# debbiemarkslab/BEAR

Measured on AMD Instinct MI355X. Metric: k-mer contexts/sec (DM-marginal+grad h), k=13, higher is better.
Workload: dtype f64

## Files before the change

### bear_amd/csrc/bear_hip.hip

```cpp
#include "bear_host.h"
#include "kernels_finalize.h"
#include "kernels_rows.h"
#include "kernels_sorted.h"
#include "kernels_plan.h"
#include "kernels_synth.h"
#include "kernels_refmix.h"
#include "kernels_mixplan.h"
#include "kernels_sample.h"
#include "kernels_shuffle.h"
#include "kernels_refplan.h"

#ifdef PLN_STAMPS
#define PLN_DBG_ARG , ws->dbg
#else
#define PLN_DBG_ARG
#endif

thread_local int g_last_hip_error = 0;

extern "C" {

int bear_abi_version(void) { return BEAR_ABI_VERSION; }

const char *bear_strerror(int status) {
// ... 451 lines not shown
  (void)hipSetDevice(prev);
  if (e != hipSuccess) {
    g_last_hip_error = (int)e;
    return BEAR_ERR_HIP;
  }
  for (uint64_t k = 0; k < count; ++k) {
    row0[k] = h[k].row0;
    rows[k] = h[k].rows_items >> 16;
    items[k] = h[k].rows_items & 0xffffu;
    stream_offset[k] = (uint64_t)h[k].off16 * 16;
  }
  return BEAR_OK;
}

int bear_plan_create_ref(bear_ws *ws, const uint32_t *train, const uint32_t *ref, uint64_t n_rows, bear_plan **out) {
  if (!out) return BEAR_ERR_INVALID_ARG;
  *out = nullptr;
  if ((n_rows && !ref) || misaligned(ref)) return BEAR_ERR_INVALID_ARG;
  bear_plan *p = nullptr;
  int st = bear_plan_create(ws, train, n_rows, 4, &p);
  if (st != BEAR_OK) return st;
  p->ref = ref;
  if (p->count_total[1] > 0.0 && (double)p->n_heavy[0] * 2.0 > p->count_total[1]) {
    (void)hipFree(p->tiles);
    (void)hipFree(p->stream);
    (void)hipFree(p->heavy_col);
    (void)hipFree(p->heavy_row);
    (void)hipFree(p->heavy_stop);
    p->tiles = nullptr;
    p->stream = nullptr;
    p->heavy_col = nullptr;
    p->heavy_row = nullptr;
    p->heavy_stop = nullptr;
    p->n_tiles = 0;
    p->n_heavy[0] = p->n_heavy[1] = p->n_heavy[2] = 0;
    p->rows_ref = 1;
    p->bytes = sizeof(unsigned long long) * (2 * SRT_NKEY + PLN_NBIG + 1);
    *out = p;
    return BEAR_OK;
  }
  unsigned long long *d_meta = nullptr;
  hipError_t e = hipMalloc(&d_meta, sizeof(unsigned long long) * 72);
  if (e == hipSuccess) e = hipMemset(d_meta, 0, sizeof(unsigned long long) * 72);
  if (e == hipSuccess) e = hipMalloc(&p->sum0, sizeof(double));
  if (e == hipSuccess) e = hipMemset(p->sum0, 0, sizeof(double));
  p->hist0_base = d_meta;
  unsigned long long h_meta[72];
  memset(h_meta, 0, sizeof(h_meta));
  const int grid = grid_capped((n_rows + 1023) / 1024, (uint64_t)ws->num_cu * 8);
  if (e == hipSuccess && n_rows) {
    hipLaunchKernelGGL(rpl_build_kernel, dim3(grid), dim3(256), 0, 0, train, ref, n_rows, 0, d_meta, d_meta + 32, d_meta + 64, p->sum0,
                       static_cast<rpl_item *>(nullptr), static_cast<uint32_t *>(nullptr));
    e = hipGetLastError();
    if (e == hipSuccess) e = hipMemcpy(h_meta, d_meta, sizeof(h_meta), hipMemcpyDeviceToHost);
  }
  if (e == hipSuccess) {
    unsigned long long run = 0, cur[RPL_NKEY];
    for (int k = 0; k < RPL_NKEY; ++k) {
      cur[k] = run;
      run += h_meta[k];
    }
    p->n_ref_items = run;
    p->n_heavy0 = h_meta[64];
    if (run) e = hipMalloc(&p->ref_items, sizeof(rpl_item) * run);
    if (e == hipSuccess && p->n_heavy0) e = hipMalloc(&p->heavy0, sizeof(uint32_t) * p->n_heavy0);
    if (e == hipSuccess) e = hipMemcpy(d_meta, cur, sizeof(cur), hipMemcpyHostToDevice);
    if (e == hipSuccess) e = hipMemset(d_meta + 64, 0, sizeof(unsigned long long));
    if (e == hipSuccess && n_rows && (run || p->n_heavy0)) {
      hipLaunchKernelGGL(rpl_build_kernel, dim3(grid), dim3(256), 0, 0, train, ref, n_rows, 1, d_meta, d_meta + 32, d_meta + 64, p->sum0,
                         p->ref_items, p->heavy0);
      e = hipGetLastError();
    }
    if (e == hipSuccess) e = hipDeviceSynchronize();
#ifdef BEAR_DET_BUILD
    for (int k = 0; k < RPL_NKEY && e == hipSuccess; ++k)
      if (bear_canonical_order(p->ref_items + cur[k], h_meta[k], 16, 0) != BEAR_OK) e = hipErrorUnknown;
    if (e == hipSuccess && bear_canonical_order(p->heavy0, p->n_heavy0, 4, 0) != BEAR_OK) e = hipErrorUnknown;
#endif
  }
  if (e != hipSuccess) {
    g_last_hip_error = (int)e;
    plan_free(p);
    return e == hipErrorOutOfMemory ? BEAR_ERR_NOMEM : BEAR_ERR_HIP;
  }
  p->hist0 = d_meta + 32;
  p->bytes += sizeof(rpl_item) * p->n_ref_items + sizeof(uint32_t) * p->n_heavy0 + sizeof(unsigned long long) * 72;
  *out = p;
  return BEAR_OK;
}

static int launch_prior_plan(bear_ws *ws, const bear_plan *plan, const double *prior, uint64_t n_rows, const bear_params &prm,
                             const double *theta, int train_ar, int prior_normalized, double *out, hipStream_t s) {
  const int grid = grid_plan(ws, plan->n_tiles);
  const double2 *lt = reinterpret_cast<const double2 *>(ws->logtab);
  const bear_step_io io = ws_io(ws, theta, BEAR_THETA_NET, out);
  if (train_ar)
    hipLaunchKernelGGL((dm_prior_plan_kernel<true, true>), dim3(grid), dim3(PLN_THREADS), sizeof(pln_lds_n), s, prior, n_rows, prm,
                       plan_view(plan), lt, ws->partials, io PLN_DBG_ARG);
  else if (prior_normalized)
    hipLaunchKernelGGL((dm_prior_plan_kernel<true, false>), dim3(grid), dim3(PLN_THREADS), sizeof(pln_lds_n), s, prior, n_rows, prm,
                       plan_view(plan), lt, ws->partials, io PLN_DBG_ARG);
  else
    hipLaunchKernelGGL((dm_prior_plan_kernel<false, false>), dim3(grid), dim3(PLN_THREADS), sizeof(pln_lds_n), s, prior, n_rows, prm,
                       plan_view(plan), lt, ws->partials, io PLN_DBG_ARG);
  HIP_TRY(hipGetLastError());
  return BEAR_OK;
}

int bear_dm_prior_plan_f64(bear_ws *ws, const bear_plan *plan, const uint32_t *counts, const double *prior,
                           uint64_t n_rows, double h_signed, double eps, int train_ar, int prior_normalized,
                           double *out, void *stream) {
  int st = check_ws(ws);
  if (st != BEAR_OK) return st;
  if (!plan || !out || (n_rows && (!counts || !prior))) return BEAR_ERR_INVALID_ARG;
  if (check_plan_step(ws, plan, counts, n_rows, 5, true) != BEAR_OK || misaligned(prior) || misaligned8(out)) return BEAR_ERR_INVALID_ARG;
  const bear_params prm = params_net(h_signed, eps);
  if (plan_is_rows(plan)) return launch_prior_rows(ws, plan, prior, prm, nullptr, train_ar, out, nullptr, static_cast<hipStream_t>(stream));
  return launch_prior_plan(ws, plan, prior, n_rows, prm, nullptr, train_ar, prior_normalized, out, static_cast<hipStream_t>(stream));
}

int launch_prior_plan_grad(bear_ws *ws, const bear_plan *plan, const double *prior, const bear_params &prm,
                                  const double *theta, int train_ar, int prior_normalized, double *out, double *grad_prior,
                                  hipStream_t s) {
  const int grid = grid_plan(ws, plan->n_tiles);
  const double2 *lt = reinterpret_cast<const double2 *>(ws->logtab);
  const pln_view pv = plan_view(plan);
  const bear_step_io io = ws_io(ws, theta, BEAR_THETA_NET, out);
  if (train_ar)
    hipLaunchKernelGGL((dm_prior_plan_grad_kernel<true, true>), dim3(grid), dim3(PLN_THREADS), sizeof(pln_lds_g), s, prior, prm, pv, lt,
                       grad_prior, ws->partials, io);
  else if (prior_normalized)
    hipLaunchKernelGGL(dm_prior_plan_grad_inplace_kernel, dim3(grid), dim3(PLN_THREADS), sizeof(pln_lds_gi), s, prior, prm, pv, lt,
                       grad_prior, ws->partials, io);
  else
    hipLaunchKernelGGL((dm_prior_plan_grad_kernel<false, false>), dim3(grid), dim3(PLN_THREADS), sizeof(pln_lds_g), s, prior, prm, pv, lt,
                       grad_prior, ws->partials, io);
  HIP_TRY(hipGetLastError());
  auto fixup_grid = [&](uint64_t nh) { return grid_capped((nh + 255) / 256, (uint64_t)ws->num_cu * 8); };
#define FIXUP(NORM, AR, ROWS, N) \
  hipLaunchKernelGGL((dm_prior_grad_fixup_kernel<NORM, AR, ROWS>), dim3(fixup_grid(N)), dim3(256), 0, s, prior, prm, pv, lt, grad_prior, io)
  if (pv.n_heavy_row && !train_ar) {
    if (prior_normalized) FIXUP(true, false, true, pv.n_heavy_row);
    else FIXUP(false, false, true, pv.n_heavy_row);
  }
  if (pv.n_heavy_col) {
    if (train_ar) FIXUP(true, true, false, pv.n_heavy_col);
    else if (prior_normalized) FIXUP(true, false, false, pv.n_heavy_col);
    else FIXUP(false, false, false, pv.n_heavy_col);
  }
#undef FIXUP
  HIP_TRY(hipGetLastError());
  return BEAR_OK;
}

int bear_dm_prior_plan_grad_f64(bear_ws *ws, const bear_plan *plan, const uint32_t *counts, const double *prior,
                                uint64_t n_rows, double h_signed, double eps, int train_ar, int prior_normalized,
                                double *out, double *grad_prior, void *stream) {
  int st = check_ws(ws);
  if (st != BEAR_OK) return st;
  if (!plan || !out || !grad_prior || (n_rows && (!counts || !prior))) return BEAR_ERR_INVALID_ARG;
  if (check_plan_step(ws, plan, counts, n_rows, 5, true) != BEAR_OK) return BEAR_ERR_INVALID_ARG;
  if (misaligned(prior) || misaligned(grad_prior) || misaligned8(out)) return BEAR_ERR_INVALID_ARG;
  const bear_params prm = params_net(h_signed, eps);
  if (plan_is_rows(plan)) return launch_prior_rows(ws, plan, prior, prm, nullptr, train_ar, out, grad_prior, static_cast<hipStream_t>(stream));
  return launch_prior_plan_grad(ws, plan, prior, prm, nullptr, train_ar, prior_normalized, out, grad_prior,
                                static_cast<hipStream_t>(stream));
}

int bear_dm_prior_plan_dev_f64(bear_ws *ws, const bear_plan *plan, const uint32_t *counts, const double *prior, uint64_t n_rows,
                               const double *h_signed_dev, double eps, int train_ar, int prior_normalized, double *out,
                               double *grad_prior, void *stream) {
  int st = check_ws(ws);
  if (st != BEAR_OK) return st;
  if (!plan || !out || !h_signed_dev || (n_rows && (!counts || !prior))) return BEAR_ERR_INVALID_ARG;
  if (check_plan_step(ws, plan, counts, n_rows, 5, true) != BEAR_OK) return BEAR_ERR_INVALID_ARG;
  if (misaligned(prior) || misaligned(grad_prior) || misaligned8(out)) return BEAR_ERR_INVALID_ARG;
  hipStream_t s = static_cast<hipStream_t>(stream);
  const bear_params only_eps = params_eps(eps);
  if (plan_is_rows(plan)) return launch_prior_rows(ws, plan, prior, only_eps, h_signed_dev, train_ar, out, grad_prior, s);
  if (grad_prior) return launch_prior_plan_grad(ws, plan, prior, only_eps, h_signed_dev, train_ar, prior_normalized, out, grad_prior, s);
  return launch_prior_plan(ws, plan, prior, n_rows, only_eps, h_signed_dev, train_ar, prior_normalized, out, s);
}

int bear_dm_refmix_plan_grad_f64(bear_ws *ws, const bear_plan *plan, const uint32_t *counts, const double *net_rows,
                                 const double *ref_rows, uint64_t n_rows, const double *h_signed_dev, const double *tau_signed_dev,
                                 const double *net_weight_signed_dev, double eps, int train_ar, double *out, double *grad_net_rows,
                                 void *stream) {
  int st = check_ws(ws);
  if (st != BEAR_OK) return st;
  if (!plan || !out || !h_signed_dev || !tau_signed_dev || !net_weight_signed_dev) return BEAR_ERR_INVALID_ARG;
  if (n_rows && (!counts || !net_rows || !ref_rows || !grad_net_rows)) return BEAR_ERR_INVALID_ARG;
  if (check_plan_step(ws, plan, counts, n_rows, 5) != BEAR_OK) return BEAR_ERR_INVALID_ARG;
  if (misaligned(net_rows) || misaligned(ref_rows) || misaligned(grad_net_rows) || misaligned8(out) || misaligned8(h_signed_dev) ||
      misaligned8(tau_signed_dev) || misaligned8(net_weight_signed_dev) || !(eps >= 0.0))
    return BEAR_ERR_INVALID_ARG;
  hipStream_t s = static_cast<hipStream_t>(stream);
  const int grid = grid_plan(ws, plan->n_tiles);
  const double2 *lt = reinterpret_cast<const double2 *>(ws->logtab);
  const pln_view pv = plan_view(plan);
  const bear_step_io io = ws_io(ws, nullptr, BEAR_THETA_REF, out);
#define MIX_LAUNCH(AR)                                                                                                            \
  hipLaunchKernelGGL(dm_refmix_plan_grad_kernel<AR>, dim3(grid), dim3(PLN_THREADS), sizeof(pln_lds_g), s, net_rows, ref_rows, \
                     h_signed_dev, tau_signed_dev, net_weight_signed_dev, eps, pv, lt, grad_net_rows, ws->partials, io)
  BEAR_DISPATCH_1(train_ar, MIX_LAUNCH);
#undef MIX_LAUNCH
  HIP_TRY(hipGetLastError());
  if (pv.n_heavy_col + pv.n_heavy_row) {
    const uint64_t nh = pv.n_heavy_col + pv.n_heavy_row;
    const int g2 = grid_capped((nh + 255) / 256, (uint64_t)ws->num_cu * 4);
#define MIX_FIXUP(AR)                                                                                                      \
  hipLaunchKernelGGL(dm_refmix_fixup_kernel<AR>, dim3(g2), dim3(256), 0, s, net_rows, ref_rows, h_signed_dev, tau_signed_dev, \
                     net_weight_signed_dev, eps, pv, lt, grad_net_rows)
    BEAR_DISPATCH_1(train_ar, MIX_FIXUP);
#undef MIX_FIXUP
    HIP_TRY(hipGetLastError());
  }
  return BEAR_OK;
}


static int launch_ref_plan(bear_ws *ws, const bear_plan *plan, const uint32_t *ref, uint64_t n_rows, const bear_params &prm,
                           const double *theta, int train_ar, double *out, hipStream_t s, const bear_apply_io &apply = NO_APPLY) {
  const double2 *lt = reinterpret_cast<const double2 *>(ws->logtab);
  const bear_step_io io = ws_io(ws, theta, BEAR_THETA_REF, out);
  int grid;
  if (plan->rows_ref) {
    if (plan->ref != ref) return BEAR_ERR_INVALID_ARG;
    grid = grid_dense(ws, n_rows);
#define REF_ROWS(AR) \
  hipLaunchKernelGGL(dm_ref_rows_kernel<AR>, dim3(grid), dim3(BEAR_THREADS), 0, s, plan->counts, ref, n_rows, prm, lt, ws->partials, io, apply)
    BEAR_DISPATCH_1(train_ar, REF_ROWS);
#undef REF_ROWS
  } else if (plan->ref) {
    if (plan->ref != ref) return BEAR_ERR_INVALID_ARG;
    rpl_view rv;
    rv.items = plan->ref_items;
    rv.n_items = plan->n_ref_items;
    rv.hist0 = plan->hist0;
    rv.heavy0 = plan->heavy0;
    rv.n_heavy0 = plan->n_heavy0;
    rv.sum0 = plan->sum0;
    const uint64_t units = (plan->n_ref_items + 63) / 64, want = (units + 3) / 4 + 2, cap = (uint64_t)ws->num_cu * (units > 131072 ? 6 : 4);
    grid = grid_capped(want, cap);
#define REF_ITEMS(AR) \
  hipLaunchKernelGGL(dm_ref_items_kernel<AR>, dim3(grid), dim3(256), 0, s, prm, rv, plan_view(plan), lt, ws->partials, io, apply)
    BEAR_DISPATCH_1(train_ar, REF_ITEMS);
#undef REF_ITEMS
  } else {
    grid = grid_plan(ws, plan->n_tiles);
#define REF_PLAN(AR)                                                                                                                     \
  hipLaunchKernelGGL(dm_ref_plan_kernel<AR>, dim3(grid), dim3(PLN_THREADS), sizeof(pln_lds_r), s, ref, n_rows, prm, plan_view(plan), lt, \
                     ws->partials, io, apply)
    BEAR_DISPATCH_1(train_ar, REF_PLAN);
#undef REF_PLAN
  }
  HIP_TRY(hipGetLastError());
  return BEAR_OK;
}

int bear_dm_ref_plan_f64(bear_ws *ws, const bear_plan *plan, const uint32_t *train, const uint32_t *ref,
                         uint64_t n_rows, double h_signed, double tau_signed, double nu_signed, double eps,
                         int train_ar, double *out, void *stream) {
  int st = check_ws(ws);
  if (st != BEAR_OK) return st;
  if (!plan || !out || (n_rows && (!train || !ref))) return BEAR_ERR_INVALID_ARG;
  if (check_plan_step(ws, plan, train, n_rows, 4) != BEAR_OK || misaligned(ref) || misaligned8(out)) return BEAR_ERR_INVALID_ARG;
  return launch_ref_plan(ws, plan, ref, n_rows, params_ref(h_signed, tau_signed, nu_signed, eps), nullptr, train_ar, out,
                         static_cast<hipStream_t>(stream));
}

static int ref_reduce(bear_ws *ws, const bear_plan *plan, const uint32_t *train, const uint32_t *ref, uint64_t n_rows, const double *theta,
                      double eps, int train_ar, double *packed, hipStream_t s, const bear_apply_io &apply) {
  int st = check_ws(ws);
  if (st != BEAR_OK) return st;
  if (!plan || !packed || !theta || !n_rows || !train || !ref) return BEAR_ERR_INVALID_ARG;
  if (check_plan_step(ws, plan, train, n_rows, 4) != BEAR_OK || misaligned(ref) || misaligned8(packed)) return BEAR_ERR_INVALID_ARG;
  return launch_ref_plan(ws, plan, ref, n_rows, params_eps(eps), theta, train_ar, packed, s, apply);
}

int bear_ref_train_reduce_f64(bear_ws *ws, const bear_plan *plan, const uint32_t *train, const uint32_t *ref, uint64_t n_rows,
                              const double *theta, double eps, int train_ar, double *packed, void *stream) {
  return ref_reduce(ws, plan, train, ref, n_rows, theta, eps, train_ar, packed, static_cast<hipStream_t>(stream), NO_APPLY);
}

int bear_ref_train_step_f64(bear_ws *ws, const bear_plan *plan, const uint32_t *train, const uint32_t *ref, uint64_t n_rows,
                            double *theta, double *adam_m, double *adam_v, double *adam_t, double eps, int train_ar,
                            double learning_rate, double scale, double *out, double *loss_buf, uint64_t loss_cap, void *stream) {
  if (!adam_m || !adam_v || !adam_t) return BEAR_ERR_INVALID_ARG;
  hipStream_t s = static_cast<hipStream_t>(stream);
  if (two_launch_step()) {
    int st = ref_reduce(ws, plan, train, ref, n_rows, theta, eps, train_ar, out, s, NO_APPLY);
    if (st != BEAR_OK) return st;
    return launch_train_apply(theta, 3, out, adam_m, adam_v, adam_t, learning_rate, scale, train_ar, loss_buf, loss_cap, s);
  }
  return ref_reduce(ws, plan, train, ref, n_rows, theta, eps, train_ar, out, s,
                    make_apply(theta, 3, adam_m, adam_v, adam_t, learning_rate, scale, train_ar, loss_buf, loss_cap));
}

int bear_dm_items_f64(bear_ws *ws, const double *x, const uint32_t *c, uint64_t n, int path, double *D, double *P,
                      void *stream) {
  int st = check_ws(ws);
  if (st != BEAR_OK) return st;
  if (n == 0) return BEAR_OK;
  if (!x || !c || !D || !P || path < 0 || path > 2) return BEAR_ERR_INVALID_ARG;
  uint64_t blocks = (n + 255) / 256;
  if (blocks > 0x7fffffffull) return BEAR_ERR_INVALID_ARG;
  hipLaunchKernelGGL(dm_items_kernel, dim3((unsigned)blocks), dim3(256), 0, static_cast<hipStream_t>(stream), x, c, n, path,
                     reinterpret_cast<const double2 *>(ws->logtab), D, P);
  HIP_TRY(hipGetLastError());
  return BEAR_OK;
}

int bear_plan_count_total(const bear_plan *plan, double *total, double *bound) {
  if (!plan) return BEAR_ERR_INVALID_ARG;
  for (int k = 0; k < 3; ++k) {
    if (total) total[k] = plan->count_total[k];
    if (bound) bound[k] = plan->count_bound[k];
  }
  return BEAR_OK;
}

int bear_plan_set_count_bound(bear_plan *plan, const double *bound) {
  if (!plan || !bound) return BEAR_ERR_INVALID_ARG;
  for (int k = 0; k < 3; ++k)
    if (!(bound[k] >= plan->count_total[k]) || !(bound[k] < 0x1p50)) return BEAR_ERR_INVALID_ARG;
  for (int k = 0; k < 3; ++k) plan->count_bound[k] = bound[k];
  return BEAR_OK;
}

static int refmix_grid(const bear_ws *ws, uint64_t n_rows) { return grid_capped((n_rows + RMX_THREADS - 1) / RMX_THREADS, ws_blocks(ws, 2)); }

int bear_ref_mix_forward_f64(bear_ws *ws, const double *net_rows, const double *ref_rows, uint64_t n_rows, const double *tau_signed,
                             const double *net_weight_signed, double *prior, void *stream) {
  int st = check_ws(ws);
  if (st != BEAR_OK) return st;
  if (!tau_signed || !net_weight_signed || misaligned8(tau_signed) || misaligned8(net_weight_signed)) return BEAR_ERR_INVALID_ARG;
  if (n_rows == 0) return BEAR_OK;
  if (!net_rows || !ref_rows || !prior || misaligned(net_rows) || misaligned(ref_rows) || misaligned(prior)) return BEAR_ERR_INVALID_ARG;
  hipLaunchKernelGGL(ref_mix_forward_kernel, dim3(refmix_grid(ws, n_rows)), dim3(RMX_THREADS), 0, static_cast<hipStream_t>(stream),
                     net_rows, ref_rows, tau_signed, net_weight_signed, n_rows, prior);
  HIP_TRY(hipGetLastError());
  return BEAR_OK;
}

int bear_ref_mix_backward_f64(bear_ws *ws, const double *net_rows, const double *ref_rows, const double *grad_prior, uint64_t n_rows,
                              const double *tau_signed, const double *net_weight_signed, double *grad_net_rows, double *grad_scalars,
                              void *stream) {
  int st = check_ws(ws);
  if (st != BEAR_OK) return st;
  if (!tau_signed || !net_weight_signed || !grad_scalars || misaligned8(tau_signed) || misaligned8(net_weight_signed) ||
      misaligned8(grad_scalars))
    return BEAR_ERR_INVALID_ARG;
  hipStream_t s = static_cast<hipStream_t>(stream);
  if (n_rows == 0) {
    HIP_TRY(hipMemsetAsync(grad_scalars, 0, 2 * sizeof(double), s));
    return BEAR_OK;
  }
  if (!net_rows || !ref_rows || !grad_prior || !grad_net_rows || misaligned(net_rows) || misaligned(ref_rows) ||
      misaligned(grad_prior) || misaligned(grad_net_rows))
    return BEAR_ERR_INVALID_ARG;
  hipLaunchKernelGGL(ref_mix_backward_kernel, dim3(refmix_grid(ws, n_rows)), dim3(RMX_THREADS), 0, s, net_rows, ref_rows, grad_prior,
                     tau_signed, net_weight_signed, n_rows, grad_net_rows, ws->partials, ws_arrival(ws), grad_scalars);
  HIP_TRY(hipGetLastError());
  return BEAR_OK;
}

int bear_debug_read_timing(bear_ws *ws, unsigned long long *host, int n_words) {
  if (!ws || !host) return BEAR_ERR_INVALID_ARG;
  HIP_TRY(hipDeviceSynchronize());
  HIP_TRY(hipMemcpy(host, ws->dbg, sizeof(unsigned long long) * (size_t)n_words, hipMemcpyDeviceToHost));
  return BEAR_OK;
}

int bear_debug_occupancy(int which) {
  int nb = -1;
  hipError_t e = which == 0
      ? hipOccupancyMaxActiveBlocksPerMultiprocessor(&nb, dm_prior_sorted_kernel<0>, SRT_THREADS, sizeof(srt_lds_n))
      : hipOccupancyMaxActiveBlocksPerMultiprocessor(&nb, dm_ref_sorted_kernel, SRT_THREADS, sizeof(srt_lds_r));
  return e == hipSuccess ? nb : -1000 - (int)e;
}

int bear_log_gamma_f64(const double *conc, uint64_t n, uint64_t n_samples, uint64_t seed, double *out, void *stream) {
  if (n == 0 || n_samples == 0) return BEAR_OK;
  if (!conc || !out) return BEAR_ERR_INVALID_ARG;
  if (n_samples > (~0ull) / n) return BEAR_ERR_INVALID_ARG;
  const uint64_t total = n * n_samples;
  uint64_t blocks = (total + SMP_THREADS - 1) / SMP_THREADS;
  if (blocks > 65536) blocks = 65536;
  hipLaunchKernelGGL(log_gamma_kernel, dim3((unsigned)blocks), dim3(SMP_THREADS), 0, static_cast<hipStream_t>(stream), conc, n,
                     n_samples, seed, out);
  HIP_TRY(hipGetLastError());
  return BEAR_OK;
}

static int logdir_sample_launch(const uint32_t *counts, const double *prior, uint64_t n_rows, int width, const double *h,
                                int n_h, int with_ar, const double *van, int n_van, int mc_samples, int map, uint64_t seed,
                                uint64_t row_base, double *out, void *stream) {
  if (n_h < 0 || n_van < 0 || n_h + n_van > SMP_MAX_MODELS || (n_h && !h) || (n_van && !van)) return BEAR_ERR_INVALID_ARG;
  if (with_ar && !map) return BEAR_ERR_INVALID_ARG;
  if (map) mc_samples = 1;
  if (mc_samples <= 0) return BEAR_ERR_INVALID_ARG;
  const int M = (with_ar ? 1 : 0) + n_h + n_van;
  if (n_rows == 0 || M == 0) return BEAR_OK;
  if (!out || ((n_h || with_ar) && !prior)) return BEAR_ERR_INVALID_ARG;
  smp_args A;
  memset(&A, 0, sizeof(A));
  A.n_h = n_h;
  A.n_van = n_van;
  A.arm = with_ar ? 1 : 0;
  A.has_counts = counts ? 1 : 0;
  A.has_prior = prior ? 1 : 0;
  A.map = map ? 1 : 0;
  A.mc = (uint32_t)mc_samples;
  A.seed = seed;
  A.row_base = row_base;
  for (int j = 0; j < n_h; ++j) {
    if (!(h[j] > 0.0)) return BEAR_ERR_INVALID_ARG;
    A.w[j] = 1.0 / h[j];
  }
  for (int k = 0; k < n_van; ++k) A.w[n_h + k] = van[k];
  const uint64_t per_row = (uint64_t)M * (uint64_t)mc_samples;
  if (per_row > 0xffffffffull || n_rows > (~0ull) / ((uint64_t)width * per_row)) return BEAR_ERR_INVALID_ARG;
  uint64_t blocks = (n_rows * per_row + SMP_THREADS - 1) / SMP_THREADS;
  if (blocks > 65536) blocks = 65536;
  hipStream_t s = static_cast<hipStream_t>(stream);
  if (width == 21)
    hipLaunchKernelGGL(logdir_sample_kernel<21>, dim3((unsigned)blocks), dim3(SMP_THREADS), 0, s, counts, prior, n_rows, A, out);
  else
    hipLaunchKernelGGL(logdir_sample_kernel<5>, dim3((unsigned)blocks), dim3(SMP_THREADS), 0, s, counts, prior, n_rows, A, out);
  HIP_TRY(hipGetLastError());
  return BEAR_OK;
}

int bear_logdir_sample_f64(const uint32_t *counts, const double *prior, uint64_t n_rows, const double *h, int n_h,
                           int with_ar, const double *van, int n_van, int mc_samples, int map, uint64_t seed,
                           uint64_t row_base, double *out, void *stream) {
  return logdir_sample_launch(counts, prior, n_rows, 5, h, n_h, with_ar, van, n_van, mc_samples, map, seed, row_base, out, stream);
}

int bear_logdir_sample_wide_f64(const uint32_t *counts, const double *prior, uint64_t n_rows, int width, const double *h,
                                int n_h, int with_ar, const double *van, int n_van, int mc_samples, int map, uint64_t seed,
                                uint64_t row_base, double *out, void *stream) {
  if (!wide_width_ok(width)) return BEAR_ERR_INVALID_ARG;
  return logdir_sample_launch(counts, prior, n_rows, width, h, n_h, with_ar, van, n_van, mc_samples, map, seed, row_base, out,
                              stream);
}

int bear_shuffle_rows(const void *src, void *dst, uint64_t n_rows, uint32_t row_bytes, uint64_t seed, void *stream) {
  if (n_rows == 0 || row_bytes == 0) return BEAR_OK;
  if (!src || !dst || src == dst) return BEAR_ERR_INVALID_ARG;
  if (n_rows > (1ull << 62) / row_bytes) return BEAR_ERR_INVALID_ARG;
  const uint32_t hb = shf_half_bits(n_rows);
  const bool words = (row_bytes % 4 == 0) && ((reinterpret_cast<uintptr_t>(src) | reinterpret_cast<uintptr_t>(dst)) % 4 == 0);
  const uint64_t total = words ? n_rows * (row_bytes / 4) : n_rows * (uint64_t)row_bytes;
  uint64_t blocks = (total + 255) / 256;
  if (blocks > 1u << 20) blocks = 1u << 20;
  if (words)
    hipLaunchKernelGGL(shuffle_words_kernel, dim3((unsigned)blocks), dim3(256), 0, static_cast<hipStream_t>(stream),
                       static_cast<const uint32_t *>(src), static_cast<uint32_t *>(dst), n_rows, row_bytes / 4, hb, seed);
  else
    hipLaunchKernelGGL(shuffle_bytes_kernel, dim3((unsigned)blocks), dim3(256), 0, static_cast<hipStream_t>(stream),
                       static_cast<const uint8_t *>(src), static_cast<uint8_t *>(dst), n_rows, row_bytes, hb, seed);
  HIP_TRY(hipGetLastError());
  return BEAR_OK;
}

uint64_t bear_shuffle_source_row(uint64_t i, uint64_t n_rows, uint64_t seed) {
  return (n_rows == 0 || i >= n_rows) ? i : shf_perm(i, n_rows, shf_half_bits(n_rows), seed);
}

int bear_stream_read(bear_ws *ws, const void *src, uint64_t n_bytes, void *stream) {
  int st = check_ws(ws);
  if (st != BEAR_OK) return st;
  if (!src || misaligned(src)) return BEAR_ERR_INVALID_ARG;
  hipLaunchKernelGGL(stream_read_kernel, dim3(ws->num_cu * 16), dim3(256), 0, static_cast<hipStream_t>(stream),
                     static_cast<const uint4 *>(src), n_bytes / 16, reinterpret_cast<uint32_t *>(ws->dbg));
  HIP_TRY(hipGetLastError());
  return BEAR_OK;
}

int bear_synth_counts_u32(uint64_t seed, uint64_t row0, uint64_t n_rows, int dense, uint32_t *train,
                          uint32_t *test, uint32_t *ref, void *stream) {
  if (n_rows == 0) return BEAR_OK;
  if (!train && !test && !ref) return BEAR_ERR_INVALID_ARG;
  uint64_t blocks = (n_rows + 255) / 256;
  if (blocks > 0x7fffffffull) return BEAR_ERR_INVALID_ARG;
  hipLaunchKernelGGL(synth_counts_kernel, dim3((unsigned)blocks), dim3(256), 0, static_cast<hipStream_t>(stream), seed, row0, n_rows, dense, train, test, ref);
  HIP_TRY(hipGetLastError());
  return BEAR_OK;
}

int bear_synth_prior_f64(uint64_t seed, uint64_t row0, uint64_t n_rows, double *prior, void *stream) {
  if (n_rows == 0) return BEAR_OK;
  if (!prior) return BEAR_ERR_INVALID_ARG;
  uint64_t blocks = (n_rows + 255) / 256;
  if (blocks > 0x7fffffffull) return BEAR_ERR_INVALID_ARG;
  hipLaunchKernelGGL(synth_prior_kernel, dim3((unsigned)blocks), dim3(256), 0, static_cast<hipStream_t>(stream), seed, row0, n_rows, prior);
  HIP_TRY(hipGetLastError());
  return BEAR_OK;
}

}
```

### bear_amd/csrc/bear_math.h

```cpp
#pragma once
#include <hip/hip_runtime.h>
#include <stdint.h>

#define BEAR_KPROD 16u
#define BEAR_TSTIR 8.0

struct bear_dp {
  double D;
  double P;
};

__device__ __forceinline__ double bear_rcp(double x) {
  double r = __builtin_amdgcn_rcp(x);
  double e = __builtin_fma(-x, r, 1.0);
  r = __builtin_fma(r, e, r);
  e = __builtin_fma(-x, r, 1.0);
  r = __builtin_fma(r, e, r);
  return r;
}

__device__ __forceinline__ double bear_log(double x) { return log(x); }

__device__ __forceinline__ double bear_log1p_pos(double t) {
  double u = 1.0 + t;
  double d = t - (u - 1.0);
  return bear_log(u) + d * bear_rcp(u);
}

__device__ __forceinline__ double bear_stir_lg(double r) {
  double r2 = r * r;
  double s = 1.0 / 156.0;
  s = __builtin_fma(s, r2, -691.0 / 360360.0);
  s = __builtin_fma(s, r2, 1.0 / 1188.0);
  s = __builtin_fma(s, r2, -1.0 / 1680.0);
  s = __builtin_fma(s, r2, 1.0 / 1260.0);
  s = __builtin_fma(s, r2, -1.0 / 360.0);
  s = __builtin_fma(s, r2, 1.0 / 12.0);
  return s * r;
}

__device__ __forceinline__ double bear_stir_psi(double r) {
  double r2 = r * r;
  double s = 1.0 / 12.0;
  s = __builtin_fma(s, r2, -691.0 / 32760.0);
  s = __builtin_fma(s, r2, 1.0 / 132.0);
  s = __builtin_fma(s, r2, -1.0 / 240.0);
  s = __builtin_fma(s, r2, 1.0 / 252.0);
  s = __builtin_fma(s, r2, -1.0 / 120.0);
  s = __builtin_fma(s, r2, 1.0 / 12.0);
  return s * r2;
}

__device__ __forceinline__ bear_dp bear_stirling_diff(double y, double c) {
  double y1 = y + c;
  double ry = bear_rcp(y), ry1 = bear_rcp(y1);
  double l1p = bear_log1p_pos(c * ry);
  double ly = bear_log(y);
  bear_dp o;
  o.D = __builtin_fma(y1 - 0.5, l1p, c * (ly - 1.0)) + (bear_stir_lg(ry1) - bear_stir_lg(ry));
  o.P = l1p - 0.5 * (ry1 - ry) - (bear_stir_psi(ry1) - bear_stir_psi(ry));
  return o;
}

__device__ __forceinline__ bear_dp bear_dm_item(double x, double c) {
  uint32_t m;
  if (c > (double)BEAR_KPROD || x > 0x1p60) {
    double need = BEAR_TSTIR - x;
    m = need > 0.0 ? (uint32_t)ceil(need) : 0u;
  } else {
    m = (uint32_t)c;
  }
  double p = 1.0, dp = 0.0, t = x;
  for (uint32_t j = 0; j < m; ++j) {
    dp = __builtin_fma(dp, t, p);
    p *= t;
    t += 1.0;
  }
  bear_dp o;
  o.D = 0.0;
  o.P = 0.0;
  if (m > 0) {
    o.D = bear_log(p);
    o.P = dp * bear_rcp(p);
  }
  if ((double)m < c) {
    bear_dp s = bear_stirling_diff(t, c - (double)m);
    o.D += s.D;
    o.P += s.P;
  }
  return o;
}

__device__ __forceinline__ double bear_fma3(double a, double b, double c) {
  double r;
  asm("v_fma_f64 %0, %1, %2, %3" : "=v"(r) : "v"(a), "v"(b), "v"(c));
  return r;
}
template <bool COEF_V = false>
__device__ __forceinline__ double bear_log1p_small(double t) {
  double q;
  if (COEF_V) asm("v_fma_f64 %0, %1, %2, %3" : "=v"(q) : "v"(-1.0 / 6.0), "v"(t), "v"(0.2));
  else asm("v_fma_f64 %0, %1, %2, %3" : "=v"(q) : "s"(-1.0 / 6.0), "v"(t), "v"(0.2));
  q = __builtin_fma(q, t, -0.25);
  q = bear_fma3(q, t, 1.0 / 3.0);
  q = __builtin_fma(q, t, -0.5);
  return __builtin_fma(t * t, q, t);
}

#define BEAR_LOGTAB_N 128
template <bool COEF_V = false>
__device__ __forceinline__ double bear_log_tab(double p, const double2 *__restrict__ tab) {
  const double m = __builtin_amdgcn_frexp_mant(p);
  const int e = __builtin_amdgcn_frexp_exp(p);
  const uint32_t hi = (uint32_t)(__double_as_longlong(m) >> 32);
  const double2 rl = tab[(hi >> 13) & 127u];
  const double t = __builtin_fma(m, rl.x, -1.0);
  const double l1p = bear_log1p_small<COEF_V>(t);
  return __builtin_fma((double)e, 0.6931471805599453094, rl.y + l1p);
}


__device__ __forceinline__ bear_dp bear_dm_item_fast(double x, double c, const double2 *__restrict__ tab) {
  uint32_t m;
  const bool stir = c > (double)BEAR_KPROD || x > 0x1p60;
  if (stir) {
    const double need = BEAR_TSTIR - x;
    m = need > 0.0 ? (uint32_t)ceil(need) : 0u;
  } else {
    m = (uint32_t)c;
  }
  double p = 1.0, dp = 0.0, t = x;
  for (uint32_t j = 0; j < m; ++j) {
    dp = __builtin_fma(dp, t, p);
    p *= t;
    t += 1.0;
  }
  bear_dp o;
  o.D = 0.0;
  o.P = 0.0;
  if (m > 0) {
    o.D = bear_log_tab(p, tab);
    o.P = dp * bear_rcp(p);
  }
  if (stir) {
    const double y = t, cc = c - (double)m, y1 = y + cc;
    const double ry = bear_rcp(y), ry1 = bear_rcp(y1);
    const double r = cc * ry;
    const double ly = bear_log_tab(y, tab);
    const double u1 = 1.0 + r;
    const double l1p = r < 0x1p-8 ? bear_log1p_small(r) : __builtin_fma(r - (u1 - 1.0), bear_rcp(u1), bear_log_tab(u1, tab));
    o.D += __builtin_fma(y1 - 0.5, l1p, cc * (ly - 1.0)) + (bear_stir_lg(ry1) - bear_stir_lg(ry));
    o.P += l1p - 0.5 * (ry1 - ry) - (bear_stir_psi(ry1) - bear_stir_psi(ry));
  }
  return o;
}

#define BEAR_EXPTAB_N 128
__device__ __forceinline__ double bear_exp_tab(double z, const double *__restrict__ tab) {
  if (z < -700.0) return 0.0;
  const double kf = __builtin_rint(z * 184.66496523378731);
  double r = __builtin_fma(kf, -0x1.62e42fee00000p-8, z);
  r = __builtin_fma(kf, -0x1.a39ef35793c76p-40, r);
  const int ki = (int)kf;
  const double t = tab[ki & (BEAR_EXPTAB_N - 1)];
  double p = __builtin_fma(r, 1.0 / 120.0, 1.0 / 24.0);
  p = __builtin_fma(r, p, 1.0 / 6.0);
  p = __builtin_fma(r, p, 0.5);
  p = __builtin_fma(r, p, 1.0);
  const double v = __builtin_fma(t, r * p, t);
  return __longlong_as_double(__double_as_longlong(v) + ((long long)(ki >> 7) << 52));
}

template <int CTRL>
__device__ __forceinline__ double bear_dpp_mov(double v) {
  const long long q = __double_as_longlong(v);
  const int lo = __builtin_amdgcn_mov_dpp((int)(uint32_t)q, CTRL, 0xf, 0xf, true);
  const int hi = __builtin_amdgcn_mov_dpp((int)(uint32_t)(q >> 32), CTRL, 0xf, 0xf, true);
  return __longlong_as_double(((long long)hi << 32) | (uint32_t)lo);
}
__device__ __forceinline__ double bear_wave_sum(double v) {
  v += bear_dpp_mov<0xB1>(v);
  v += bear_dpp_mov<0x4E>(v);
  v += bear_dpp_mov<0x124>(v);
  v += bear_dpp_mov<0x128>(v);
#pragma unroll
  for (int step = 0; step < 2; ++step) {
    const long long q = __double_as_longlong(v);
    const uint32_t lo = (uint32_t)q, hi = (uint32_t)(q >> 32);
    const auto a = step == 0 ? __builtin_amdgcn_permlane16_swap(lo, lo, false, false) : __builtin_amdgcn_permlane32_swap(lo, lo, false, false);
    const auto c = step == 0 ? __builtin_amdgcn_permlane16_swap(hi, hi, false, false) : __builtin_amdgcn_permlane32_swap(hi, hi, false, false);
    v = __longlong_as_double(((long long)c[0] << 32) | a[0]) + __longlong_as_double(((long long)c[1] << 32) | a[1]);
  }
  return v;
}
__device__ __forceinline__ double bear_wave_max(double v) {
  v = __builtin_fmax(v, bear_dpp_mov<0xB1>(v));
  v = __builtin_fmax(v, bear_dpp_mov<0x4E>(v));
  v = __builtin_fmax(v, bear_dpp_mov<0x124>(v));
  v = __builtin_fmax(v, bear_dpp_mov<0x128>(v));
#pragma unroll
  for (int step = 0; step < 2; ++step) {
    const long long q = __double_as_longlong(v);
    const uint32_t lo = (uint32_t)q, hi = (uint32_t)(q >> 32);
    const auto a = step == 0 ? __builtin_amdgcn_permlane16_swap(lo, lo, false, false) : __builtin_amdgcn_permlane32_swap(lo, lo, false, false);
    const auto c = step == 0 ? __builtin_amdgcn_permlane16_swap(hi, hi, false, false) : __builtin_amdgcn_permlane32_swap(hi, hi, false, false);
    v = __builtin_fmax(__longlong_as_double(((long long)c[0] << 32) | a[0]), __longlong_as_double(((long long)c[1] << 32) | a[1]));
  }
  return v;
}
```

### bear_amd/csrc/kernels_rows.h

```cpp
#pragma once
#include "bear_common.h"

template <int NT = BEAR_THREADS>
__device__ __forceinline__ void stage_dwords(uint32_t *lds, const uint32_t *src, uint32_t n_dwords) {
  const uint32_t n_vec = n_dwords >> 2;
  const uint4 *s4 = reinterpret_cast<const uint4 *>(src);
  uint4 *d4 = reinterpret_cast<uint4 *>(lds);
  for (uint32_t i = threadIdx.x; i < n_vec; i += NT) d4[i] = s4[i];
  for (uint32_t i = (n_vec << 2) + threadIdx.x; i < n_dwords; i += NT) lds[i] = src[i];
}

template <int TILE, typename TB, typename Row>
__device__ __forceinline__ void for_row_tiles(uint64_t n_rows, const uint32_t *a, uint32_t *s_a, const TB *b, TB *s_b, Row row) {
  const uint64_t n_tiles = (n_rows + TILE - 1) / TILE;
  for (uint64_t tile = blockIdx.x; tile < n_tiles; tile += gridDim.x) {
    const uint64_t row0 = tile * TILE;
    const uint32_t rows = (uint32_t)((n_rows - row0 < TILE) ? (n_rows - row0) : TILE);
    __syncthreads();
    stage_dwords(s_a, a + row0 * 5, rows * 5);
    stage_dwords(reinterpret_cast<uint32_t *>(s_b), reinterpret_cast<const uint32_t *>(b + row0 * 5), rows * (5 * sizeof(TB) / 4));
    __syncthreads();
#pragma unroll 1
    for (int k = 0; k < TILE / BEAR_THREADS; ++k) {
      const uint32_t r = threadIdx.x + k * BEAR_THREADS;
      if (r >= rows) break;
      row(row0, r);
    }
  }
}

__device__ __forceinline__ bear_dp dm_row_item(double x, double c, const double2 *tab) {
  if (tab && x > 0.0 && x < INFINITY) return bear_dm_item_fast(x, c, tab);
  return bear_dm_item(x, c);
}
__device__ __forceinline__ double dm_row(const uint32_t (&c)[5], const double (&a)[5], double (&g)[5], const double2 *tab = nullptr) {
  const double n = (((double)c[0] + (double)c[1]) + ((double)c[2] + (double)c[3])) + (double)c[4];
  double ll = 0.0;
#pragma unroll
  for (int b = 0; b < 5; ++b) g[b] = 0.0;
  if (n == 0.0) return 0.0;
  double A = ((a[0] + a[1]) + (a[2] + a[3])) + a[4];
  bear_dp tn = dm_row_item(A, n, tab);
  ll = -tn.D;
#pragma unroll
  for (int b = 0; b < 5; ++b) {
    g[b] = -tn.P;
    if (c[b] != 0) {
      bear_dp tb = dm_row_item(a[b], (double)c[b], tab);
      ll += tb.D;
      g[b] += tb.P;
    }
  }
  return ll;
}

template <bool AR, bool GRAD>
__device__ __forceinline__ void dm_prior_row(const uint32_t *s_cnt, const double *s_pri, uint32_t r, const bear_params &prm,
                                             double *grad_row, const double2 *s_log, double (&acc)[2]) {
  uint32_t c[5];
  double f[5];
#pragma unroll
  for (int b = 0; b < 5; ++b) {
    c[b] = s_cnt[r * 5 + b];
    f[b] = s_pri[r * 5 + b];
  }
  if (AR) {
#pragma unroll
    for (int b = 0; b < 5; ++b) {
      const double p = f[b] + prm.eps, cb = (double)c[b];
      if (c[b] != 0) acc[0] += cb * (p > 0.0 ? bear_log_tab(p, s_log) : bear_log(p));
      if (GRAD) grad_row[b] = c[b] != 0 ? cb * bear_rcp(p) : 0.0;
    }
  } else {
    double a[5], g[5];
#pragma unroll
    for (int b = 0; b < 5; ++b) a[b] = __builtin_fma(f[b], prm.inv_h, prm.eps);
    acc[0] += dm_row(c, a, g, s_log);
    double dh = 0.0;
#pragma unroll
    for (int b = 0; b < 5; ++b) {
      dh = __builtin_fma(g[b], f[b], dh);
      if (GRAD) grad_row[b] = g[b] * prm.inv_h;
    }
    acc[1] -= dh * prm.inv_h;
  }
}

template <bool AR, bool TAB>
__device__ __forceinline__ void dm_ref_row(const uint32_t *s_trn, const uint32_t *s_ref, uint32_t r, const bear_params &prm,
                                           const double2 *s_log, double (&acc)[4]) {
  uint32_t c[5];
  double rr[4];
#pragma unroll
  for (int b = 0; b < 5; ++b) c[b] = s_trn[r * 5 + b];
#pragma unroll
  for (int b = 0; b < 4; ++b) rr[b] = (double)s_ref[r * 5 + b] + prm.eps;
  const double invR = bear_rcp((rr[0] + rr[1]) + (rr[2] + rr[3]));
  double f[5], dft[5], dfn[5];
#pragma unroll
  for (int b = 0; b < 4; ++b) {
    const double dev = __builtin_fma(rr[b], invR, -0.25);
    f[b] = __builtin_fma(prm.E, dev, 0.25) * prm.V;
    dft[b] = -prm.tauE * dev * prm.V;
    dfn[b] = -prm.nw * f[b] * prm.V;
  }
  f[4] = prm.nw * prm.V;
  dft[4] = 0.0;
  dfn[4] = prm.nw * (1.0 - f[4]) * prm.V;
  double dLdf[5];
  if (AR) {
#pragma unroll
    for (int b = 0; b < 5; ++b) {
      const double p = f[b] + prm.eps, cb = (double)c[b];
      dLdf[b] = 0.0;
      if (c[b] != 0) {
        acc[0] += cb * (p > 0.0 ? bear_log_tab(p, s_log) : bear_log(p));
        dLdf[b] = cb * bear_rcp(p);
      }
    }
  } else {
    double a[5], g[5];
#pragma unroll
    for (int b = 0; b < 5; ++b) a[b] = __builtin_fma(f[b], prm.inv_h, prm.eps);
    acc[0] += TAB ? dm_row(c, a, g, s_log) : dm_row(c, a, g);
    double dh = 0.0;
#pragma unroll
    for (int b = 0; b < 5; ++b) {
      dLdf[b] = g[b] * prm.inv_h;
      dh = __builtin_fma(dLdf[b], f[b], dh);
    }
    acc[1] -= dh;
  }
#pragma unroll
  for (int b = 0; b < 5; ++b) {
    acc[2] = __builtin_fma(dLdf[b], dft[b], acc[2]);
    acc[3] = __builtin_fma(dLdf[b], dfn[b], acc[3]);
  }
}

template <bool AR, bool GRAD>
__global__ __launch_bounds__(BEAR_THREADS) void dm_prior_kernel(const uint32_t *__restrict__ counts, const double *__restrict__ prior,
                                                                 uint64_t n_rows, bear_params prm, double *__restrict__ grad_prior,
                                                                 const double2 *__restrict__ logtab_g, double *__restrict__ partials) {
  __shared__ __attribute__((aligned(16))) uint32_t s_cnt[BEAR_TILE_ROWS * 5];
  __shared__ __attribute__((aligned(16))) double s_pri[BEAR_TILE_ROWS * 5];
  __shared__ double2 s_log[BEAR_LOGTAB_N];
  if (threadIdx.x < BEAR_LOGTAB_N) s_log[threadIdx.x] = logtab_g[threadIdx.x];
  double acc[2] = {0.0, 0.0};
  for_row_tiles<BEAR_TILE_ROWS>(n_rows, counts, s_cnt, prior, s_pri, [&](uint64_t row0, uint32_t r) {
    dm_prior_row<AR, GRAD>(s_cnt, s_pri, r, prm, grad_prior + (row0 + r) * 5, s_log, acc);
  });
  block_store_partials<2>(acc, partials);
}

#ifndef DPR_TILE_ROWS
#define DPR_TILE_ROWS 512
#endif
#define DPR_BLOCKS_PER_CU 4
template <bool AR, bool GRAD>
__global__ __launch_bounds__(BEAR_THREADS, DPR_BLOCKS_PER_CU / 4) void dm_prior_rows_kernel(const uint32_t *__restrict__ counts, const double *__restrict__ prior,
                                                                      uint64_t n_rows, bear_params prm_arg, double *__restrict__ grad_prior,
                                                                      const double2 *__restrict__ logtab_g, double *__restrict__ partials,
                                                                      const bear_step_io io) {
  __shared__ __attribute__((aligned(16))) uint32_t s_cnt[DPR_TILE_ROWS * 5];
  __shared__ __attribute__((aligned(16))) double s_pri[DPR_TILE_ROWS * 5];
  __shared__ double2 s_log[BEAR_LOGTAB_N];
  const bear_params prm = bear_params_of(prm_arg, io);
  if (threadIdx.x < BEAR_LOGTAB_N) s_log[threadIdx.x] = logtab_g[threadIdx.x];
  double acc[2] = {0.0, 0.0};
  for_row_tiles<DPR_TILE_ROWS>(n_rows, counts, s_cnt, prior, s_pri, [&](uint64_t row0, uint32_t r) {
    dm_prior_row<AR, GRAD>(s_cnt, s_pri, r, prm, grad_prior + (row0 + r) * 5, s_log, acc);
  });
  __syncthreads();
  block_finish<2>(acc, partials, io);
}

template <bool AR>
__global__ __launch_bounds__(BEAR_THREADS) void dm_ref_kernel(const uint32_t *__restrict__ train, const uint32_t *__restrict__ ref,
                                                               uint64_t n_rows, bear_params prm, const double2 *__restrict__ logtab_g,
                                                               double *__restrict__ partials) {
  __shared__ double2 s_log[BEAR_LOGTAB_N];
  if (threadIdx.x < BEAR_LOGTAB_N) s_log[threadIdx.x] = logtab_g[threadIdx.x];
  __shared__ __attribute__((aligned(16))) uint32_t s_trn[BEAR_TILE_ROWS * 5];
  __shared__ __attribute__((aligned(16))) uint32_t s_ref[BEAR_TILE_ROWS * 5];
  double acc[4] = {0.0, 0.0, 0.0, 0.0};
  for_row_tiles<BEAR_TILE_ROWS>(n_rows, train, s_trn, ref, s_ref, [&](uint64_t, uint32_t r) { dm_ref_row<AR, false>(s_trn, s_ref, r, prm, s_log, acc); });
  block_store_partials<4>(acc, partials);
}

template <bool AR>
__global__ __launch_bounds__(BEAR_THREADS) void dm_ref_rows_kernel(const uint32_t *__restrict__ train, const uint32_t *__restrict__ ref,
                                                                    uint64_t n_rows, bear_params prm_arg, const double2 *__restrict__ logtab_g,
                                                                    double *__restrict__ partials, const bear_step_io io,
                                                                    const bear_apply_io apply) {
  __shared__ double2 s_log[BEAR_LOGTAB_N];
  __shared__ __attribute__((aligned(16))) uint32_t s_trn[DPR_TILE_ROWS * 5];
  __shared__ __attribute__((aligned(16))) uint32_t s_ref[DPR_TILE_ROWS * 5];
  const bear_params prm = bear_params_of(prm_arg, io);
  if (threadIdx.x < BEAR_LOGTAB_N) s_log[threadIdx.x] = logtab_g[threadIdx.x];
  double acc[4] = {0.0, 0.0, 0.0, 0.0};
  for_row_tiles<DPR_TILE_ROWS>(n_rows, train, s_trn, ref, s_ref, [&](uint64_t, uint32_t r) { dm_ref_row<AR, true>(s_trn, s_ref, r, prm, s_log, acc); });
  __syncthreads();
  block_finish<4>(acc, partials, io, apply);
}
```

Baseline: 136.9 billion.

## Add dense DM row path with hoisted per-row Stirling constants and truncated series

For the non-AR prior and ref row kernels, a dense DM path replaces the generic per-item evaluation. The row-level total term uses Stirling constants precomputed once per block from the uniform total alpha. A shortened Stirling series is used when every lane in the wave has a large argument. Per-cell evaluation shares one reciprocal across several quantities and uses log differences for large ratios. The launch bounds minimum-waves argument is also corrected to a waves-per-SIMD value. These changes cut transcendental and reciprocal work per row, at the cost of branch divergence and possible accuracy differences from the truncated series and the table-based logs.

```diff
diff --git a/bear_amd/csrc/bear_hip.hip b/bear_amd/csrc/bear_hip.hip
--- a/bear_amd/csrc/bear_hip.hip
+++ b/bear_amd/csrc/bear_hip.hip
@@ -777,11 +777,14 @@
   int st = check_ws(ws);
   if (st != BEAR_OK) return st;
   if (n == 0) return BEAR_OK;
-  if (!x || !c || !D || !P || path < 0 || path > 2) return BEAR_ERR_INVALID_ARG;
+  if (!x || !c || !D || !P || path < 0 || path > 4) return BEAR_ERR_INVALID_ARG;
   uint64_t blocks = (n + 255) / 256;
   if (blocks > 0x7fffffffull) return BEAR_ERR_INVALID_ARG;
-  hipLaunchKernelGGL(dm_items_kernel, dim3((unsigned)blocks), dim3(256), 0, static_cast<hipStream_t>(stream), x, c, n, path,
-                     reinterpret_cast<const double2 *>(ws->logtab), D, P);
+  const double2 *lt = reinterpret_cast<const double2 *>(ws->logtab);
+  hipStream_t s = static_cast<hipStream_t>(stream);
+  if (path == 3) hipLaunchKernelGGL(dm_items_dense_kernel<3>, dim3((unsigned)blocks), dim3(256), 0, s, x, c, n, lt, D, P);
+  else if (path == 4) hipLaunchKernelGGL(dm_items_dense_kernel<4>, dim3((unsigned)blocks), dim3(256), 0, s, x, c, n, lt, D, P);
+  else hipLaunchKernelGGL(dm_items_kernel, dim3((unsigned)blocks), dim3(256), 0, s, x, c, n, path, lt, D, P);
   HIP_TRY(hipGetLastError());
   return BEAR_OK;
 }
diff --git a/bear_amd/csrc/bear_math.h b/bear_amd/csrc/bear_math.h
--- a/bear_amd/csrc/bear_math.h
+++ b/bear_amd/csrc/bear_math.h
@@ -152,6 +152,100 @@
     o.D += __builtin_fma(y1 - 0.5, l1p, cc * (ly - 1.0)) + (bear_stir_lg(ry1) - bear_stir_lg(ry));
     o.P += l1p - 0.5 * (ry1 - ry) - (bear_stir_psi(ry1) - bear_stir_psi(ry));
   }
+  return o;
+}
+
+__device__ __forceinline__ double bear_stir_lg3(double r) {
+  double r2 = r * r;
+  double s = 1.0 / 1260.0;
+  s = __builtin_fma(s, r2, -1.0 / 360.0);
+  s = __builtin_fma(s, r2, 1.0 / 12.0);
+  return s * r;
+}
+__device__ __forceinline__ double bear_stir_psi3(double r) {
+  double r2 = r * r;
+  double s = 1.0 / 252.0;
+  s = __builtin_fma(s, r2, -1.0 / 120.0);
+  s = __builtin_fma(s, r2, 1.0 / 12.0);
+  return s * r2;
+}
+
+__device__ __forceinline__ bear_dp bear_dm_cell_dense(double x, double c, const double2 *__restrict__ tab) {
+  const double need = BEAR_TSTIR - x;
+  const uint32_t m = need > 0.0 ? (uint32_t)ceil(need) : 0u;
+  double p = 1.0, dp = 0.0, y = x;
+  for (uint32_t j = 0; j < m; ++j) {
+    dp = __builtin_fma(dp, y, p);
+    p *= y;
+    y += 1.0;
+  }
+  const double cc = c - (double)m, y1 = y + cc;
+  const double q = p * y;
+  const double rw = bear_rcp(q * y1);
+  const double ry1 = rw * q, rq = rw * y1;
+  const double ry = rq * p;
+  bear_dp o;
+  o.D = 0.0;
+  o.P = 0.0;
+  if (m > 0) {
+    o.D = bear_log_tab(p, tab);
+    o.P = dp * (rq * y);
+  }
+  const double r = cc * ry;
+  const double ly = bear_log_tab(y, tab);
+  double l1p;
+  if (r < 0x1p-8) {
+    l1p = bear_log1p_small(r);
+  } else {
+    const bool far = r >= 1.0;
+    const double u1 = 1.0 + r;
+    const double lt = bear_log_tab(far ? y1 : u1, tab);
+    l1p = far ? lt - ly : __builtin_fma(r - (u1 - 1.0), y * ry1, lt);
+  }
+  double tl, tp;
+  if (__builtin_amdgcn_ballot_w64(!(y1 >= 0x1p10)) == 0) {
+    tl = bear_stir_lg3(ry1);
+    tp = bear_stir_psi3(ry1);
+  } else {
+    tl = bear_stir_lg(ry1);
+    tp = bear_stir_psi(ry1);
+  }
+  o.D += __builtin_fma(y1 - 0.5, l1p, cc * (ly - 1.0)) + (tl - bear_stir_lg(ry));
+  o.P += l1p - 0.5 * (ry1 - ry) - (tp - bear_stir_psi(ry));
+  return o;
+}
+
+struct bear_row_consts {
+  double A, KD, KP;
+  bool ok;
+};
+__device__ __forceinline__ bear_row_consts bear_row_consts_of(double A) {
+  bear_row_consts k;
+  k.A = A;
+  k.ok = A >= 0x1p-300 && A < 0x1p300;
+  const double a = k.ok ? A : 1.0;
+  const double need = BEAR_TSTIR - a;
+  const uint32_t m = need > 0.0 ? (uint32_t)ceil(need) : 0u;
+  double p = 1.0, dp = 0.0, y = a;
+  for (uint32_t j = 0; j < m; ++j) {
+    dp = __builtin_fma(dp, y, p);
+    p *= y;
+    y += 1.0;
+  }
+  const double ry = bear_rcp(y), ly = bear_log(y);
+  k.KD = (__builtin_fma(y - 0.5, ly, -y) + bear_stir_lg(ry)) - bear_log(p);
+  k.KP = ((ly - 0.5 * ry) - bear_stir_psi(ry)) - dp * bear_rcp(p);
+  return k;
+}
+__device__ __forceinline__ bool bear_row_dense_ok(const bear_row_consts &k, double n) {
+  return k.ok && n >= k.A && k.A + n >= 0x1p10;
+}
+__device__ __forceinline__ bear_dp bear_row_dense(const bear_row_consts &k, double n, const double2 *__restrict__ tab) {
+  const double Y = k.A + n;
+  const double rY = bear_rcp(Y), lY = bear_log_tab(Y, tab);
+  bear_dp o;
+  o.D = (__builtin_fma(Y - 0.5, lY, -Y) + bear_stir_lg3(rY)) - k.KD;
+  o.P = ((lY - 0.5 * rY) - bear_stir_psi3(rY)) - k.KP;
   return o;
 }
 
diff --git a/bear_amd/csrc/kernels_rows.h b/bear_amd/csrc/kernels_rows.h
--- a/bear_amd/csrc/kernels_rows.h
+++ b/bear_amd/csrc/kernels_rows.h
@@ -1,5 +1,6 @@
 #pragma once
 #include "bear_common.h"
+#include "sorted_common.h"
 
 template <int NT = BEAR_THREADS>
 __device__ __forceinline__ void stage_dwords(uint32_t *lds, const uint32_t *src, uint32_t n_dwords) {
@@ -54,6 +55,45 @@
   return ll;
 }
 
+__device__ __forceinline__ bear_dp dm_dense_general(double x, double c, const double2 *tab) {
+  if (!(x > 0.0) || !(x < 0x1p1000)) return bear_dp{__builtin_nan(""), __builtin_nan("")};
+  return bear_dm_item_fast(x, c, tab);
+}
+__device__ __forceinline__ bear_dp dm_dense_item(double x, double c, const double2 *tab) {
+  if (c > (double)BEAR_KPROD && x >= 0x1p-300 && x < 0x1p300) return bear_dm_cell_dense(x, c, tab);
+  return dm_dense_general(x, c, tab);
+}
+__device__ __forceinline__ bear_row_consts dm_dense_consts(const bear_params &prm) {
+  bear_row_consts k = bear_row_consts_of(prm.inv_h + 5.0 * prm.eps);
+  k.A = bear_uniform_f64(k.A);
+  k.KD = bear_uniform_f64(k.KD);
+  k.KP = bear_uniform_f64(k.KP);
+  k.ok = __builtin_amdgcn_readfirstlane((int)k.ok) != 0;
+  return k;
+}
+template <typename Count, typename Alpha, typename Grad>
+__device__ __forceinline__ double dm_row_dense(double n, const double2 *tab, const bear_row_consts &K, bool sum1, Count count,
+                                               Alpha alpha, Grad grad) {
+  bear_dp tn{0.0, 0.0};
+  if (n != 0.0) {
+    if (sum1 && bear_row_dense_ok(K, n)) tn = bear_row_dense(K, n, tab);
+    else tn = dm_dense_general(((alpha(0) + alpha(1)) + (alpha(2) + alpha(3))) + alpha(4), n, tab);
+  }
+  double ll = 0.0 - tn.D;
+#pragma unroll
+  for (int b = 0; b < 5; ++b) {
+    double g = 0.0 - tn.P;
+    const uint32_t cb = count(b);
+    if (cb != 0) {
+      const bear_dp tb = dm_dense_item(alpha(b), (double)cb, tab);
+      ll += tb.D;
+      g += tb.P;
+    }
+    grad(b, g);
+  }
+  return ll;
+}
+
 template <bool AR, bool GRAD>
 __device__ __forceinline__ void dm_prior_row(const uint32_t *s_cnt, const double *s_pri, uint32_t r, const bear_params &prm,
                                              double *grad_row, const double2 *s_log, double (&acc)[2]) {
@@ -84,6 +124,28 @@
     }
     acc[1] -= dh * prm.inv_h;
   }
+}
+
+template <bool GRAD>
+__device__ __forceinline__ void dm_prior_row_dense(const uint32_t *s_cnt, const double *s_pri, uint32_t r, const bear_params &prm,
+                                                   double *grad_row, const double2 *s_log, const bear_row_consts &K, double (&acc)[2]) {
+  uint32_t c[5];
+  double f[5];
+#pragma unroll
+  for (int b = 0; b < 5; ++b) {
+    c[b] = s_cnt[r * 5 + b];
+    f[b] = s_pri[r * 5 + b];
+  }
+  double dh = 0.0;
+  acc[0] += dm_row_dense(
+      (((double)c[0] + (double)c[1]) + ((double)c[2] + (double)c[3])) + (double)c[4], s_log, K,
+      __builtin_fabs((((f[0] + f[1]) + (f[2] + f[3])) + f[4]) - 1.0) <= SRT_SUM1_TOL, [&](int b) { return c[b]; },
+      [&](int b) { return __builtin_fma(f[b], prm.inv_h, prm.eps); },
+      [&](int b, double g) {
+        dh = __builtin_fma(g, f[b], dh);
+        if (GRAD) grad_row[b] = g * prm.inv_h;
+      });
+  acc[1] -= dh * prm.inv_h;
 }
 
 template <bool AR, bool TAB>
@@ -136,6 +198,33 @@
     acc[2] = __builtin_fma(dLdf[b], dft[b], acc[2]);
     acc[3] = __builtin_fma(dLdf[b], dfn[b], acc[3]);
   }
+}
+__device__ __forceinline__ void dm_ref_row_dense(const uint32_t *s_trn, const uint32_t *s_ref, uint32_t r, const bear_params &prm,
+                                                 const double2 *s_log, const bear_row_consts &K, double (&acc)[4]) {
+  uint32_t c[5];
+  double rr[4], dev[4];
+#pragma unroll
+  for (int b = 0; b < 5; ++b) c[b] = s_trn[r * 5 + b];
+#pragma unroll
+  for (int b = 0; b < 4; ++b) rr[b] = (double)s_ref[r * 5 + b] + prm.eps;
+  const double invR = bear_rcp((rr[0] + rr[1]) + (rr[2] + rr[3]));
+#pragma unroll
+  for (int b = 0; b < 4; ++b) dev[b] = __builtin_fma(rr[b], invR, -0.25);
+  const double f4 = prm.nw * prm.V;
+  auto f_of = [&](int b) { return b < 4 ? __builtin_fma(prm.E, dev[b], 0.25) * prm.V : f4; };
+  double dh = 0.0;
+  acc[0] += dm_row_dense(
+      (((double)c[0] + (double)c[1]) + ((double)c[2] + (double)c[3])) + (double)c[4], s_log, K, true, [&](int b) { return c[b]; },
+      [&](int b) { return __builtin_fma(f_of(b), prm.inv_h, prm.eps); },
+      [&](int b, double g) {
+        const double fb = f_of(b), dLdf = g * prm.inv_h;
+        const double dft = b < 4 ? -prm.tauE * dev[b] * prm.V : 0.0;
+        const double dfn = b < 4 ? -prm.nw * fb * prm.V : prm.nw * (1.0 - f4) * prm.V;
+        dh = __builtin_fma(dLdf, fb, dh);
+        acc[2] = __builtin_fma(dLdf, dft, acc[2]);
+        acc[3] = __builtin_fma(dLdf, dfn, acc[3]);
+      });
+  acc[1] -= dh;
 }
 
 template <bool AR, bool GRAD>
@@ -157,8 +246,9 @@
 #define DPR_TILE_ROWS 512
 #endif
 #define DPR_BLOCKS_PER_CU 4
+#define DPR_WAVES_PER_SIMD (DPR_BLOCKS_PER_CU * (BEAR_THREADS / 64) / 4)
 template <bool AR, bool GRAD>
-__global__ __launch_bounds__(BEAR_THREADS, DPR_BLOCKS_PER_CU / 4) void dm_prior_rows_kernel(const uint32_t *__restrict__ counts, const double *__restrict__ prior,
+__global__ __launch_bounds__(BEAR_THREADS, DPR_WAVES_PER_SIMD) void dm_prior_rows_kernel(const uint32_t *__restrict__ counts, const double *__restrict__ prior,
                                                                       uint64_t n_rows, bear_params prm_arg, double *__restrict__ grad_prior,
                                                                       const double2 *__restrict__ logtab_g, double *__restrict__ partials,
                                                                       const bear_step_io io) {
@@ -168,9 +258,16 @@
   const bear_params prm = bear_params_of(prm_arg, io);
   if (threadIdx.x < BEAR_LOGTAB_N) s_log[threadIdx.x] = logtab_g[threadIdx.x];
   double acc[2] = {0.0, 0.0};
-  for_row_tiles<DPR_TILE_ROWS>(n_rows, counts, s_cnt, prior, s_pri, [&](uint64_t row0, uint32_t r) {
-    dm_prior_row<AR, GRAD>(s_cnt, s_pri, r, prm, grad_prior + (row0 + r) * 5, s_log, acc);
-  });
+  if (AR) {
+    for_row_tiles<DPR_TILE_ROWS>(n_rows, counts, s_cnt, prior, s_pri, [&](uint64_t row0, uint32_t r) {
+      dm_prior_row<true, GRAD>(s_cnt, s_pri, r, prm, grad_prior + (row0 + r) * 5, s_log, acc);
+    });
+  } else {
+    const bear_row_consts K = dm_dense_consts(prm);
+    for_row_tiles<DPR_TILE_ROWS>(n_rows, counts, s_cnt, prior, s_pri, [&](uint64_t row0, uint32_t r) {
+      dm_prior_row_dense<GRAD>(s_cnt, s_pri, r, prm, grad_prior + (row0 + r) * 5, s_log, K, acc);
+    });
+  }
   __syncthreads();
   block_finish<2>(acc, partials, io);
 }
@@ -189,7 +286,7 @@
 }
 
 template <bool AR>
-__global__ __launch_bounds__(BEAR_THREADS) void dm_ref_rows_kernel(const uint32_t *__restrict__ train, const uint32_t *__restrict__ ref,
+__global__ __launch_bounds__(BEAR_THREADS, DPR_WAVES_PER_SIMD) void dm_ref_rows_kernel(const uint32_t *__restrict__ train, const uint32_t *__restrict__ ref,
                                                                     uint64_t n_rows, bear_params prm_arg, const double2 *__restrict__ logtab_g,
                                                                     double *__restrict__ partials, const bear_step_io io,
                                                                     const bear_apply_io apply) {
@@ -199,7 +296,36 @@
   const bear_params prm = bear_params_of(prm_arg, io);
   if (threadIdx.x < BEAR_LOGTAB_N) s_log[threadIdx.x] = logtab_g[threadIdx.x];
   double acc[4] = {0.0, 0.0, 0.0, 0.0};
-  for_row_tiles<DPR_TILE_ROWS>(n_rows, train, s_trn, ref, s_ref, [&](uint64_t, uint32_t r) { dm_ref_row<AR, true>(s_trn, s_ref, r, prm, s_log, acc); });
+  if (AR) {
+    for_row_tiles<DPR_TILE_ROWS>(n_rows, train, s_trn, ref, s_ref, [&](uint64_t, uint32_t r) { dm_ref_row<true, true>(s_trn, s_ref, r, prm, s_log, acc); });
+  } else {
+    const bear_row_consts K = dm_dense_consts(prm);
+    for_row_tiles<DPR_TILE_ROWS>(n_rows, train, s_trn, ref, s_ref, [&](uint64_t, uint32_t r) { dm_ref_row_dense(s_trn, s_ref, r, prm, s_log, K, acc); });
+  }
   __syncthreads();
   block_finish<4>(acc, partials, io, apply);
 }
+
+template <int PATH>
+__global__ __launch_bounds__(256) void dm_items_dense_kernel(const double *__restrict__ x, const uint32_t *__restrict__ c, uint64_t n,
+                                                             const double2 *__restrict__ logtab_g, double *__restrict__ D,
+                                                             double *__restrict__ P) {
+  __shared__ double2 logtab[BEAR_LOGTAB_N];
+  if (threadIdx.x < BEAR_LOGTAB_N) logtab[threadIdx.x] = logtab_g[threadIdx.x];
+  __syncthreads();
+  const uint64_t i = (uint64_t)blockIdx.x * 256 + threadIdx.x;
+  if (i >= n) return;
+  const double xi = x[i], ci = (double)c[i];
+  bear_dp o{0.0, 0.0};
+  if (ci != 0.0) {
+    if (PATH == 3) {
+      o = dm_dense_item(xi, ci, logtab);
+    } else {
+      const bear_row_consts K = bear_row_consts_of(xi);
+      if (bear_row_dense_ok(K, ci)) o = bear_row_dense(K, ci, logtab);
+      else o = dm_dense_general(xi, ci, logtab);
+    }
+  }
+  D[i] = o.D;
+  P[i] = o.P;
+}
```

Result: no change. 136.9 billion (-0.0%).
